# BillyXYB/TransEditor

Measured on AMD Instinct MI355X. Metric: 256x256 images/sec/GPU, G+D fwd+bwd, batch 16; 1/2/4/8-GPU scaling, higher is better.
Workload: dtype f32

## Files before the change

include/te_hip.h:

```cpp
#ifndef TE_HIP_H
#define TE_HIP_H

#include <stdint.h>

#ifdef __cplusplus
extern "C" {
#endif

#define TE_ABI_VERSION 3

#define TE_ERR_NULL -1
#define TE_ERR_SHAPE -2
#define TE_ERR_UNSUPPORTED -3
#define TE_ERR_WORKSPACE -4

typedef void* te_stream_t;

int te_version(void);
const char* te_last_error_string(void);
const char* te_arch(void);

int te_bias_act_f32(float* out, const float* x, const float* b, const float* ref, int act, int grad,
                    float alpha, float scale, int64_t size_x, int64_t step_b, int64_t size_b,
                    te_stream_t stream);
int te_bias_act_f16(void* out, const void* x, const void* b, const void* ref, int act, int grad,
                    float alpha, float scale, int64_t size_x, int64_t step_b, int64_t size_b,
                    te_stream_t stream);
int te_bias_act_f64(double* out, const double* x, const double* b, const double* ref, int act, int grad,
                    float alpha, float scale, int64_t size_x, int64_t step_b, int64_t size_b,
                    te_stream_t stream);

int64_t te_bias_act_bwd_ws_floats(int64_t outer, int64_t C, int64_t inner);
int te_bias_act_bwd_f32(float* gi, float* gb, float* ws, const float* g, const float* ref, float alpha, float scale,
                        int64_t outer, int64_t C, int64_t inner, te_stream_t stream);
int te_bias_act_bwd_rgb_supported(int64_t outer, int64_t C, int64_t inner);
int te_bias_act_bwd_rgb_f32(float* gi, float* gb, float* ws, const float* g, const float* ref, const float* grgb, const float* wrgb,
                            const float* srgb, float wscale, float alpha, float scale, int64_t outer, int64_t C, int64_t inner,
                            te_stream_t stream);

int te_upfirdn2d_f32(float* out, const float* x, const float* k, int64_t major, int in_h, int in_w,
                     int minor, int kh, int kw, int up_x, int up_y, int down_x, int down_y, int pad_x0,
                     int pad_x1, int pad_y0, int pad_y1, const float* b, int64_t size_b, int act,
                     float alpha, float scale, te_stream_t stream);
int te_upfirdn2d_f16(void* out, const void* x, const void* k, int64_t major, int in_h, int in_w,
                     int minor, int kh, int kw, int up_x, int up_y, int down_x, int down_y, int pad_x0,
                     int pad_x1, int pad_y0, int pad_y1, te_stream_t stream);
int te_upfirdn2d_f64(double* out, const double* x, const double* k, int64_t major, int in_h, int in_w,
                     int minor, int kh, int kw, int up_x, int up_y, int down_x, int down_y, int pad_x0,
                     int pad_x1, int pad_y0, int pad_y1, te_stream_t stream);


#define TE_CONV_3X3 0
#define TE_CONV_T2 1
#define TE_CONV_S2 2
#define TE_CONV_1X1 3
#define TE_CONV_3X3W 4
#define TE_CONV_3X3W6 5

#define TE_CONV_S2S6 6

#define TE_CONV_T2S6 7

#define TE_CONV_1X1S6 8

#define TE_PACK_FWD 0
#define TE_PACK_DGRAD 1
#define TE_PACK_SWAP 2
#define TE_PACK_WFWD 3
#define TE_PACK_WDGRAD 4
#define TE_PACK_W6FWD 5
#define TE_PACK_W6DGRAD 6
#define TE_PACK_S6FWD 7
#define TE_PACK_S6SWAP 8
#define TE_PACK_T6FWD 9
#define TE_PACK_T6SWAP 10
#define TE_PACK_P6FWD 11
#define TE_PACK_P6DGRAD 12

int64_t te_conv_packed_numel(int kind_pack, int Co, int Ci, int ksize);
int te_conv_pack_weights_f32(float* wp, const float* w, float wscale, int kind_pack, int Co, int Ci,
                             int ksize, te_stream_t stream);
int te_conv_pack_weights2_f32(float* wp_a, int kind_a, float* wp_b, int kind_b, const float* w, float wscale, int Co, int Ci,
                              int ksize, te_stream_t stream);

int te_conv_pack_weights_multi_f32(int n, float* const* wp, const float* const* w, const float* wscale, const int* kind_pack,
                                   const int* Co, const int* Ci, const int* ksize, te_stream_t stream);

int te_conv_f32(float* out, const float* in, const float* wp, const float* isc, const float* osc,
                const float* bias, int act, int kind, int B, int K, int M, int H, int W,
                te_stream_t stream);
int te_conv_splitk_count(int kind, int B, int K, int M, int H, int W);
int te_conv_wino_supported(int B, int K, int M, int H, int W);
int te_conv_wino6_supported(int B, int K, int M, int H, int W);
int te_conv_s2s6_supported(int B, int K, int M, int H, int W);
int te_conv_t2s6_supported(int B, int K, int M, int H, int W);
int te_conv_p1s6_supported(int B, int K, int M, int H, int W);
int te_conv_wino6_form(int form);
int te_conv_wino6_tiles_per_block(int n);
int te_conv_s2s6_form(int form);
int te_conv_t2s6_form(int form);
int64_t te_conv_t2s6_ws_floats(int B, int K, int H);
int te_conv_ws_f32(float* out, float* ws, const float* in, const float* wp, const float* isc, const float* osc,
                   const float* bias, int act, int kind, int B, int K, int M, int H, int W, te_stream_t stream);
int te_conv_res_f32(float* out, float* ws, const float* in, const float* wp, const float* isc, const float* osc,
                    const float* bias, const float* res, const float* mask_ref, float mask_gain, int act, int kind, int B,
                    int K, int M, int H, int W, te_stream_t stream);

int te_wgrad_slab_count(int kind, int B, int Co, int Ci, int H, int W);
int te_wgrad_pair_form(int kind, int Co, int Ci, int H, int W);
int te_wgrad_split_supported(int kind, int Co, int Ci, int H, int W);
int te_wgrad_split_bf16(int on);
int te_wgrad_t2_wide(int on);
enum { TE_WG6_FP32 = 0, TE_WG6_3X3 = 1, TE_WG6_3X3_PAIR = 2, TE_WG6_T2_WIDE = 3, TE_WG6_T2 = 4, TE_WG6_T2_MASKED = 5, TE_WG6_1X1 = 6 };
int te_wgrad6_form(int kind, int B, int Co, int Ci, int H, int W, int NB);
int te_wgrad_f32(float* slabs, const float* g, const float* x, int kind, int B, int Co, int Ci, int H,
                 int W, int S, te_stream_t stream);
int te_wgrad_group_plan(int kind, int B, int Co, int Ci, int H, int W, int* NB, int* S);
int te_wgrad_group_f32(float* slabs, const float* g, const float* x, int kind, int B, int Co, int Ci, int H, int W, int S, int NB,
                       te_stream_t stream);

int64_t te_wgrad_reduce_ws_floats(int B, int S, int Co, int Ci, int taps, int want_w, int want_isc, int want_osc);
int te_wgrad_reduce_f32(float* gw, float* gisc, float* gosc, float* ws, const float* slabs, const float* w,
                        float wscale, const float* isc, const float* osc, int B, int S, int Co, int Ci,
                        int taps, te_stream_t stream);

int te_rgb_supported(int M, int K, int HW);
int te_rgb_fwd_f32(float* out, const float* x, const float* w, const float* isc, const float* bias, float wscale, int B,
                   int K, int HW, te_stream_t stream);
int te_rgb_dgrad_f32(float* gx, const float* g, const float* w, const float* isc, float wscale, int B, int K, int HW,
                     te_stream_t stream);
int te_rgb_expand_f32(float* out, const float* x3, const float* w, const float* bias, int act, float wscale, int B, int K,
                      int HW, te_stream_t stream);
int te_rgb_wgrad_slab_count(int B, int K, int HW);
int te_rgb_wgrad_f32(float* slabs, const float* g, const float* x, int B, int K, int HW, int S, te_stream_t stream);
int te_rgb_wgrad_sum_f32(float* slabs, const float* g, const float* x, int B, int K, int HW, int S, te_stream_t stream);

int te_attn_fwd_f32(float* o, float* sim, const float* q, const float* k, const float* v, float scale,
                    int N, int G, int M, int L, int D, te_stream_t stream);
int te_attn_bwd_f32(float* gq, float* gk, float* gv, const float* go, const float* gsim_or_null,
                    const float* q, const float* k, const float* v, const float* sim, float scale, int N,
                    int G, int M, int L, int D, te_stream_t stream);

int te_blur_actgrad_tiles(int in_h, int in_w, int kh, int kw, int pad_x0, int pad_x1, int pad_y0, int pad_y1);
int te_blur_actgrad_f32(float* gx, float* partial, const float* g, const float* ref, const float* k, int64_t major, int in_h,
                        int in_w, int kh, int kw, int pad_x0, int pad_x1, int pad_y0, int pad_y1, float alpha, float scale,
                        te_stream_t stream);
int te_blur_gradact_f32(float* gx, float* partial, const float* g, const float* ref, const float* k, int64_t major, int in_h,
                        int in_w, int kh, int kw, int pad_x0, int pad_x1, int pad_y0, int pad_y1, float alpha, float scale,
                        te_stream_t stream);

int te_upfirdn2d_plan(int64_t major, int in_h, int in_w, int minor, int kh, int kw, int up_x, int up_y, int down_x, int down_y,
                      int pad_x0, int pad_x1, int pad_y0, int pad_y1, int* zgroups, int* tiles);
int te_blur_actgrad_plan(int64_t major, int in_h, int in_w, int kh, int kw, int pad_x0, int pad_x1, int pad_y0, int pad_y1,
                         int* zgroups, int* tiles);
int te_blur_gradact_plan(int64_t major, int in_h, int in_w, int kh, int kw, int pad_x0, int pad_x1, int pad_y0, int pad_y1,
                         int* zgroups, int* tiles);
int64_t te_upfirdn2d_direct_cover(int64_t outputs);
int64_t te_chan_scale_cover(int64_t rows, int64_t hw, int aligned16);
int64_t te_bias_act_f32_cover(int64_t size_x, int64_t step_b, int aligned16, int* vec);
int64_t te_bias_act_any_cover(int64_t size_x);
int64_t te_conv_finalize_cover(int64_t outputs);
int64_t te_small_gemm_splitk_finish_cover(int I, int J);
int te_conv_pack_plan(int kind_pack, int Co, int Ci, int ksize, int* blocks, int* tiles);
int te_wgrad_reduce_plan(int B, int S, int Co, int Ci, int taps, int* parts, int64_t* cover);

int te_small_gemm_f32(float* c, float* pre, const float* a, const float* b, const float* bias, const float* residual,
                      float* arowsum, float rs_scale, int I, int J, int K, int64_t sai, int64_t sak, int64_t sbk,
                      int64_t sbj, float alpha, float beta, int act, te_stream_t stream);

int te_small_gemm_splitk_f32(float* c, float* pre, float* ws, int S, const float* a, const float* b, const float* bias,
                             const float* residual, int I, int J, int K, int64_t sai, int64_t sak, int64_t sbk, int64_t sbj,
                             float alpha, float beta, int act, te_stream_t stream);

int te_minibatch_stddev_fwd_f32(float* y, const float* x, int B, int group, int C, int HW, float eps, te_stream_t stream);
int te_minibatch_stddev_bwd_f32(float* gx, const float* gy, const float* x, int B, int group, int C, int HW, float eps,
                                te_stream_t stream);

int te_layer_norm_supported(int64_t R, int N);
int te_layer_norm_fwd_f32(float* y, float* stats, const float* x, int64_t R, int N, float eps, te_stream_t stream);
int te_layer_norm_bwd_f32(float* gx, const float* g, const float* y, const float* stats, int64_t R, int N, te_stream_t stream);

int te_pixel_norm_supported(int64_t B, int D, int C);
int te_pixel_norm_fwd_f32(float* y, float* r, const float* x, int64_t B, int D, int C, float eps, te_stream_t stream);
// ... 114 lines not shown
```

transeditor_amd/_lib.py:

```python
import ctypes as C
import os

import torch

from . import _abi

_HERE = os.path.dirname(os.path.abspath(__file__))
LIB_PATH = os.path.join(_HERE, 'libte_hip.so')
HEADER_PATH = os.path.join(_HERE, '..', 'include', 'te_hip.h')
_lib = _protos = None

CONV_3X3, CONV_T2, CONV_S2, CONV_1X1, CONV_3X3W, CONV_3X3W6, CONV_S2S6, CONV_T2S6, CONV_1X1S6 = 0, 1, 2, 3, 4, 5, 6, 7, 8
(PACK_FWD, PACK_DGRAD, PACK_SWAP, PACK_WFWD, PACK_WDGRAD, PACK_W6FWD, PACK_W6DGRAD, PACK_S6FWD, PACK_S6SWAP, PACK_T6FWD,
 PACK_T6SWAP, PACK_P6FWD, PACK_P6DGRAD) = range(13)


def _header_text():
    if not os.path.exists(HEADER_PATH):
        raise RuntimeError(f'{HEADER_PATH} is missing: the bindings of libte_hip.so are read from it')
    with open(HEADER_PATH) as f:
        return f.read()


def _prototypes():
# ... 195 lines not shown
    B, Cn, H, W = g.shape
    kh, kw = k_flipped.shape
    px0, px1, py0, py1 = pad
    oh, ow = H + py0 + py1 - kh + 1, W + px0 + px1 - kw + 1
    if tuple(ref.shape) != (B, Cn, oh, ow):
        raise RuntimeError(f'blur_gradact: ref {tuple(ref.shape)} is not the shape of the adjoint blur output {(B, Cn, oh, ow)}')
    tiles = lib().te_blur_actgrad_tiles(H, W, kh, kw, px0, px1, py0, py1)
    if tiles <= 0:
        raise RuntimeError(f'te_blur_actgrad_tiles failed ({tiles})')
    gx = torch.empty(B, Cn, oh, ow, device=g.device, dtype=g.dtype)
    partial = torch.empty(B, Cn, tiles, device=g.device, dtype=g.dtype)
    _launch('te_blur_gradact_f32', _ptr(gx), _ptr(partial), _ptr(g), _ptr(ref), _ptr(k_flipped.contiguous()), B * Cn, H, W, kh, kw, px0,
            px1, py0, py1, alpha, scale)
    return gx, partial.sum(dim=(0, 2))


@_op
def conv_pack(w, kind_pack, wscale=1.0):
    w = w.contiguous()
    Co, Ci, ks, _ = w.shape
    n = lib().te_conv_packed_numel(kind_pack, Co, Ci, ks)
    wp = torch.empty(n, device=w.device, dtype=w.dtype)
    _launch('te_conv_pack_weights_f32', _ptr(wp), _ptr(w), wscale, kind_pack, Co, Ci, ks)
    return wp


@_op
def conv_pack2(w, kind_a, kind_b, wscale=1.0):
    w = w.contiguous()
    Co, Ci, ks, _ = w.shape
    wa = torch.empty(lib().te_conv_packed_numel(kind_a, Co, Ci, ks), device=w.device, dtype=w.dtype)
    wb = torch.empty(lib().te_conv_packed_numel(kind_b, Co, Ci, ks), device=w.device, dtype=w.dtype)
    _launch('te_conv_pack_weights2_f32', _ptr(wa), kind_a, _ptr(wb), kind_b, _ptr(w), wscale, Co, Ci, ks)
    return wa, wb


@_op
def conv_pack_multi(jobs):
    n = len(jobs)
    if not n:
        return
    for wp, w, _, _ in jobs:
        if not (w.is_contiguous() and wp.is_contiguous()):
            raise RuntimeError('te_hip: conv_pack_multi needs dense weights and buffers')
    arr = lambda ty, vals: (ty * n)(*vals)
    _launch('te_conv_pack_weights_multi_f32', n, arr(C.c_void_p, [_ptr(j[0]) for j in jobs]), arr(C.c_void_p, [_ptr(j[1]) for j in jobs]),
            arr(C.c_float, [float(j[3]) for j in jobs]), arr(C.c_int, [int(j[2]) for j in jobs]),
            arr(C.c_int, [j[1].shape[0] for j in jobs]), arr(C.c_int, [j[1].shape[1] for j in jobs]),
            arr(C.c_int, [j[1].shape[2] for j in jobs]))


def wino_ok(B, K, M, H, W):
    return bool(lib().te_conv_wino_supported(B, K, M, H, W))


def s2s6_ok(B, K, M, H, W):
    return bool(lib().te_conv_s2s6_supported(B, K, M, H, W))


def t2s6_ok(B, K, M, H, W):
    return bool(lib().te_conv_t2s6_supported(B, K, M, H, W))


def p1s6_ok(B, K, M, H, W):
    return bool(lib().te_conv_p1s6_supported(B, K, M, H, W))


def wino6_form(form=-1):
    return int(lib().te_conv_wino6_form(form))


def wino6_tiles_per_block(n=-1):
    return int(lib().te_conv_wino6_tiles_per_block(n))


def s2s6_form(form=-1):
    return int(lib().te_conv_s2s6_form(form))


def t2s6_form(form=-1):
    return int(lib().te_conv_t2s6_form(form))


def wino6_ok(B, K, M, H, W):
    return bool(lib().te_conv_wino6_supported(B, K, M, H, W))


def conv_out_shape(kind, B, M, H, W):
    if kind in (CONV_T2, CONV_T2S6):
        return (B, M, 2 * H + 1, 2 * W + 1)
    return (B, M, H, W)


@_op
def conv(x, wp, kind, M, H, W, isc=None, osc=None, bias=None, act=0, res=None, mask_ref=None, mask_gain=1.0):
    x = x.contiguous()
    if kind == CONV_1X1S6:
        x = _aligned16(x)
    res = _aligned16(res.contiguous()) if res is not None else None
    mask_ref = _aligned16(mask_ref.contiguous()) if mask_ref is not None else None
    B, K = x.shape[0], x.shape[1]
    out = torch.empty(conv_out_shape(kind, B, M, H, W), device=x.device, dtype=x.dtype)
    if res is not None and tuple(res.shape) != tuple(out.shape):
        raise RuntimeError(f'te_hip: residual {tuple(res.shape)} does not match the convolution output {tuple(out.shape)}')
    if mask_ref is not None and tuple(mask_ref.shape) != tuple(out.shape):
        raise RuntimeError(f'te_hip: mask reference {tuple(mask_ref.shape)} does not match the convolution output {tuple(out.shape)}')
    S = lib().te_conv_splitk_count(kind, B, K, M, H, W)
    if S < 1:
        raise RuntimeError(f'te_conv_splitk_count failed ({S})')
    ws = torch.empty((S,) + tuple(out.shape), device=x.device, dtype=x.dtype) if S > 1 else None
    if kind == CONV_T2S6:
        ws = torch.empty(B * K * H, device=x.device, dtype=x.dtype)
    _launch('te_conv_res_f32', _ptr(out), _ptr(ws), _ptr(x), _ptr(wp), _ptr(isc), _ptr(osc), _ptr(bias), _ptr(res), _ptr(mask_ref),
            mask_gain, act, kind, B, K, M, H, W)
    return out


@_op
def wgrad_slabs(g, x, kind, H, W, group=False):
    g, x = g.contiguous(), x.contiguous()
    B, Co, Ci = g.shape[0], g.shape[1], x.shape[1]
    taps = 1 if kind == CONV_1X1 else 9
    if group:
        nb, sc = C.c_int(0), C.c_int(0)
        _check(lib().te_wgrad_group_plan(kind, B, Co, Ci, H, W, C.byref(nb), C.byref(sc)), 'te_wgrad_group_plan')
        if nb.value > 1:
            slabs = torch.empty(B // nb.value, sc.value, Co, Ci, taps, device=g.device, dtype=g.dtype)
            _launch('te_wgrad_group_f32', _ptr(slabs), _ptr(g), _ptr(x), kind, B, Co, Ci, H, W, sc.value, nb.value)
            return slabs
    S = lib().te_wgrad_slab_count(kind, B, Co, Ci, H, W)
    if S <= 0:
        raise RuntimeError(f'te_wgrad_slab_count failed ({S})')
    slabs = torch.empty(B, S, Co, Ci, taps, device=g.device, dtype=g.dtype)
    _launch('te_wgrad_f32', _ptr(slabs), _ptr(g), _ptr(x), kind, B, Co, Ci, H, W, S)
    return slabs


def wgrad_t2_wide(on=-1):
    return int(lib().te_wgrad_t2_wide(on))


def wgrad_split(on=-1):
    return int(lib().te_wgrad_split_bf16(on))


def wgrad_split_ok(kind, Co, Ci, H, W):
    return bool(lib().te_wgrad_split_supported(kind, Co, Ci, H, W))


WGRAD6_FORMS = ('fp32', 'w6', 'w6pair', 't2wide', 't2narrow', 't2masked', 'p1')


def wgrad6_form(kind, B, Co, Ci, H, W, NB=1):
    return WGRAD6_FORMS[lib().te_wgrad6_form(kind, B, Co, Ci, H, W, NB)]


def wgrad_pair_form(kind, Co, Ci, H, W):
    return bool(lib().te_wgrad_pair_form(kind, Co, Ci, H, W))


@_op
def wgrad_reduce(slabs, w, wscale=1.0, isc=None, osc=None, want_w=True, want_isc=False, want_osc=False):
    B, S, Co, Ci, taps = slabs.shape
    dev, dt = slabs.device, slabs.dtype
    gw = torch.empty(Co, Ci, taps, device=dev, dtype=dt) if want_w else None
    gisc = torch.empty(B, Ci, device=dev, dtype=dt) if want_isc else None
# ... 873 lines not shown
```

transeditor_amd/csrc/s2s6.hip:

```cpp
#include "split6_common.h"
#ifdef S2_PROF
#define TE_PROF
#endif
#include "te_prof.h"

namespace {

constexpr int WT = 512, GT = 256, KC = 16, BM = 64;
constexpr int TH = 8, TWO = 16, PH = 4;
constexpr int IR = 2 * PH + 1, IC = 2 * TWO + 1;
constexpr int CI = 18;
constexpr int NTAP = 9;
constexpr int U_SLOTS = 3 * NTAP * 2;
constexpr int TP_PLANE = IR * 2 * 2 * CI * 4;
constexpr int TP_DWORDS = 3 * TP_PLANE;
constexpr int NG = (IC + 3) / 4;
constexpr int N_ITEMS = IR * NG * 8;
constexpr int P_IN = (N_ITEMS + GT - 1) / GT;
constexpr int N_SLOT = P_IN + 16 * P_IN;
constexpr int SLOT0 = NTAP * 6 - N_SLOT;
constexpr int UA_TAPS = 5;

PROF_BUFFER(s2s6, 2048 * 8 * 8)

struct S2Args {
    float* out; const float* in; const u32x4* U; const float* isc; const float* osc; const float* bias; const float* res;
    const float* mref; float mgain; int act;
    int B, K, M, H, W, Hi, Wi, ntiles, mblocks, tiles_x, tiles_y, nt8;
};


template <bool ISC, bool TWOIMG>
__device__ __attribute__((optnone)) void s2s6_body(const S2Args& p) {
    constexpr int NIMG = TWOIMG ? 2 : 1;
    extern __shared__ __attribute__((aligned(16))) unsigned char smem_raw[];
    u32x4* ul = reinterpret_cast<u32x4*>(smem_raw);
    const int tid = threadIdx.x, lane = tid & 63, l31 = lane & 31, half = lane >> 5;
    const int wid = __builtin_amdgcn_readfirstlane(tid >> 6);
    const int grp = wid >> 2, wq = wid & 3, wm = wq >> 1, wrl = wq & 1, gt = tid & (GT - 1);
    unsigned* tl = reinterpret_cast<unsigned*>(smem_raw + U_SLOTS * 1024) + grp * TP_DWORDS;
    const u32x4* tl4 = reinterpret_cast<const u32x4*>(tl);
    int tile, mbq;
    if (!split6_tile(p.ntiles, p.nt8, p.mblocks, tile, mbq)) return;
    const int tx = tile % p.tiles_x, ty = (tile / p.tiles_x) % p.tiles_y, b = tile / (p.tiles_x * p.tiles_y);
    const int x0 = tx * TWO, y0 = ty * TH, yh = y0 + PH * grp;
    const size_t iplane = (size_t)p.Hi * p.Wi, oplane = (size_t)p.H * p.W;
    const float* inb = p.in + (size_t)b * p.K * iplane;
    const float* iscb = ISC ? p.isc + (size_t)b * p.K : nullptr;

    f32x16 acc[NIMG], accl[NIMG];
#pragma unroll
    for (int m = 0; m < NIMG; ++m)
#pragma unroll
        for (int r = 0; r < 16; ++r) { acc[m][r] = 0.f; accl[m][r] = 0.f; }

    unsigned g_off[P_IN];
    int l_off[P_IN];
    bool last_col[P_IN], live[P_IN];
    unsigned q2[P_IN];
#pragma unroll
    for (int i = 0; i < P_IN; ++i) {
        const int e = gt + GT * i;
        live[i] = e < N_ITEMS;
        const int ee = live[i] ? e : 0;
        const int cg = ee % NG, q = (ee / NG) & 7, row = ee / (NG * 8);
        last_col[i] = cg == NG - 1;
        g_off[i] = (unsigned)((2 * q * p.Hi + 2 * yh + row) * p.Wi + 2 * x0 + 4 * cg - (last_col[i] ? 3 : 0));
        l_off[i] = (((row * 2 + (q >> 2)) * 2) * CI + 2 * cg) * 4 + (q & 3);
        q2[i] = 2u * q;
    }
    const int MT = p.M >> 5;
    f32x4 rin[P_IN][2];
    f32x2 rsc[P_IN];
#pragma unroll
    for (int i = 0; i < P_IN; ++i) rsc[i] = f32x2{1.f, 1.f};
    const int nstage = p.K / KC, nimg = NIMG * nstage;
    auto fetch_scales = [&](int s) {
        if (ISC) {
#pragma unroll
            for (int i = 0; i < P_IN; ++i) rsc[i] = *reinterpret_cast<const f32x2u*>(iscb + s * KC + q2[i]);
        }
    };
    auto fetch_item = [&](int i, int s) {
#pragma unroll
        for (int h2 = 0; h2 < 2; ++h2)
            rin[i][h2] = *reinterpret_cast<const f32x4u*>(inb + ((size_t)s * KC + h2) * iplane + g_off[i]);
    };
    auto issue = [&](int s) {
        fetch_scales(s);
#pragma unroll
        for (int i = 0; i < P_IN; ++i) fetch_item(i, s);
    };
    auto issue_u = [&](int uh, int j) {
        const u32x4* us = p.U + (size_t)(TWOIMG ? j >> 1 : j) * 27 * MT * 64;
        const int mb = TWOIMG ? 2 * mbq + (j & 1) : mbq;
        const int ntap = uh ? NTAP - UA_TAPS : UA_TAPS, tap0 = uh ? UA_TAPS : 0, n = ntap * 6;
#pragma unroll
        for (int r = 0; r < 8; ++r) {
            const int jw = wq + 4 * r;
            if (jw >= n) break;
            const int piece = jw / (ntap * 2), rem = jw % (ntap * 2), tap = tap0 + (rem >> 1), mt = rem & 1;
            const int pt = piece * NTAP + tap;
            const u32x4* g = us + ((size_t)pt * MT + 2 * mb + mt) * 64 + (unsigned)lane;
            __builtin_amdgcn_global_load_lds((const __attribute__((address_space(1))) void*)g,
                                             (__attribute__((address_space(3))) void*)(ul + (pt * 2 + mt) * 64), 16, 0, 0);
        }
    };
    unsigned res[P_IN][4][3];
    float te = 0.f, to = 0.f, fe = 0.f, fo = 0.f;
    auto arith = [&](int k) {
        if (k < 0) {
        } else if (k < P_IN) {
#pragma unroll
            for (int h2 = 0; h2 < 2; ++h2) {
                f32x4 v = rin[k][h2];
                if (last_col[k]) v[0] = v[3];
                rin[k][h2] = ISC ? v * rsc[k][h2] : v;
                asm volatile("" : "+v"(rin[k][h2]));
            }
        } else if (k < N_SLOT) {
            const int u = (k - P_IN) >> 2, j = (k - P_IN) & 3, i = u >> 2, c = u & 3;
            float ve = 0.f, vo = 0.f;
            if (j == 0) {
                ve = rin[i][0][c]; vo = rin[i][1][c];
            }
            split6_step4(j, ve, vo, te, to, fe, fo, res[i][c][0], res[i][c][1], res[i][c][2]);
        }
    };
    auto write_res = [&]() {
#pragma unroll
        for (int i = 0; i < P_IN; ++i) {
            if (!live[i]) continue;
#pragma unroll
            for (int c = 0; c < 4; ++c) {
                if (c > 0 && last_col[i]) continue;
#pragma unroll
                for (int pc = 0; pc < 3; ++pc) tl[l_off[i] + (c & 1) * CI * 4 + (c >> 1) * 4 + pc * TP_PLANE] = res[i][c][pc];
            }
        }
    };
    const int rr = l31 >> 4, jj = l31 & 15;
    const int b_chunk = ((2 * (2 * wrl + rr) * 2 + half) * 2) * CI + jj;
    const int a_chunk = wm * 64 + lane;
    bf16x8 av[2][3], bv[2][3];
    auto rd1 = [&](int t, int slot, int q) {
        const int ky = t / 3, kx = t % 3;
        if (q < 3) av[slot][q] = __builtin_bit_cast(bf16x8, ul[a_chunk + (q * NTAP + t) * 128]);
        else bv[slot][q - 3] = __builtin_bit_cast(bf16x8, tl4[b_chunk + ((ky * 2) * 2 + (kx & 1)) * CI + (kx >> 1) + (q - 3) * (TP_PLANE / 4)]);
    };

    issue(0);
    if (grp == 0) { issue_u(0, 0); issue_u(1, 0); }
#pragma unroll
    for (int k = 0; k < N_SLOT; ++k) arith(k);
    write_res();
    if constexpr (!TWOIMG) {
        issue(1);
        if (grp == 0) {
            if (ISC) asm volatile("s_waitcnt vmcnt(9)" ::: "memory");
            else asm volatile("s_waitcnt vmcnt(6)" ::: "memory");
        }
        split6_barrier();
        const int nphase = 2 * nstage;
        PROF_ONLY(unsigned long long pc[8] = {0, 0, 0, 0, 0, 0, 0, 0};)
        PROF_ONLY(const unsigned long long pstart = __builtin_readcyclecounter(), rstart = __builtin_amdgcn_s_memrealtime();)
        for (int ph = 0; ph < nphase; ++ph) {
            const bool last = ph == nphase - 1;
            PROF_T(t0);
            if ((ph & 1) == grp) {
                const int fs2 = min((ph >> 1) + 2, nstage - 1);
#pragma unroll
                for (int q = 0; q < 6; ++q) rd1(0, 0, q);
                __builtin_amdgcn_s_setprio(1);
#pragma unroll
                for (int t = 0; t < NTAP; ++t) {
                    const int slot = t & 1;
                    if (t == UA_TAPS - 1) { PROF_T(ta); split6_barrier(); PROF_T(tb); PROF_ACC(pc[0], t0, ta); PROF_ACC(pc[1], ta, tb); PROF_ONLY(pc[2] -= tb;) }
                    __builtin_amdgcn_sched_barrier(0);
#pragma unroll
                    for (int q = 0; q < 6; ++q) {
                        split6_product(q, av[slot], bv[slot], acc[0], accl[0]);
                        if (t + 1 < NTAP && q < 3) { rd1(t + 1, slot ^ 1, 2 * q); rd1(t + 1, slot ^ 1, 2 * q + 1); }
                        arith(t * 6 + q - SLOT0);
                        {
                            const int k = t * 6 + q - SLOT0;
                            if (k == P_IN - 1) fetch_scales(fs2);
#pragma unroll
                            for (int i = 0; i < P_IN; ++i)
                                if (k == P_IN + 16 * i + 12) fetch_item(i, fs2);
                        }
                        __builtin_amdgcn_sched_barrier(0);
                    }
                }
                __builtin_amdgcn_s_setprio(0);
                PROF_ONLY({ asm volatile("s_nop 0" ::: "memory"); PROF_T(tc); pc[2] += tc; })
            } else {
                const int cs = (ph + 1) >> 1;
                const bool work = cs >= 1 && cs < nimg;
                if (work && grp == 1) issue_u(1, cs);
                __builtin_amdgcn_sched_barrier(0);
                write_res();
                if (work && grp == 1) split6_wait_vm();
                PROF_T(ta);
                split6_barrier();
                PROF_T(tb);
                if (work && grp == 0) {
                    issue_u(0, cs);
                    split6_wait_vm();
                }
                PROF_T(tc);
                PROF_ACC(pc[3], t0, ta); PROF_ACC(pc[4], ta, tb); PROF_ACC(pc[5], tb, tc);
            }
            PROF_T(t8);
            if (!last) split6_barrier();
            PROF_T(t9);
            PROF_ACC(pc[6], t8, t9);
        }
        PROF_ONLY(if (lane == 0 && blockIdx.x < 2048) {
            unsigned long long* d = te_s2s6_prof_buf + ((size_t)blockIdx.x * 8 + wid) * 8;
            _Pragma("unroll")
            for (int i = 0; i < 6; ++i) d[i] = pc[i];
            d[6] = pc[6] | ((__builtin_amdgcn_s_memrealtime() - rstart) << 40);
            d[7] = ((unsigned long long)nstage << 48) | ((__builtin_readcyclecounter() - pstart) & 0xFFFFFFFFFFFFull);
        })
    } else {
        auto multiply = [&](auto mset_tag, int fs) {
            constexpr int MSET = decltype(mset_tag)::value;
#pragma unroll
            for (int q = 0; q < 6; ++q) rd1(0, 0, q);
            __builtin_amdgcn_s_setprio(1);
#pragma unroll
            for (int t = 0; t < NTAP; ++t) {
                const int slot = t & 1;
                if (t == UA_TAPS - 1) split6_barrier();
                __builtin_amdgcn_sched_barrier(0);
#pragma unroll
                for (int q = 0; q < 6; ++q) {
                    split6_product(q, av[slot], bv[slot], acc[MSET], accl[MSET]);
                    if (t + 1 < NTAP && q < 3) { rd1(t + 1, slot ^ 1, 2 * q); rd1(t + 1, slot ^ 1, 2 * q + 1); }
                    const int k = t * 6 + q;
                    if (MSET == 0) {
                        if (k == 5) fetch_scales(fs);
#pragma unroll
                        for (int i = 0; i < P_IN; ++i)
                            if (k == 6 + 12 * i) fetch_item(i, fs);
                    } else {
                        arith(k - SLOT0);
                    }
                    __builtin_amdgcn_sched_barrier(0);
                }
            }
            __builtin_amdgcn_s_setprio(0);
            split6_barrier();
        };
        auto stage = [&](int ph, bool write) {
            const int cs = (ph + 1) >> 1;
            const bool work = cs >= 1 && cs < nimg;
            if (grp == 1 && work) issue_u(1, cs);
            __builtin_amdgcn_sched_barrier(0);
            if (write) write_res();
            if (grp == 1 && work) split6_wait_vm();
            split6_barrier();
            if (grp == 0 && work) {
                issue_u(0, cs);
                split6_wait_vm();
            }
            split6_barrier();
        };
        split6_wait_vm();
        split6_barrier();
        int ph = 0;
        if (grp == 1) { stage(0, false); ph = 1; }
        for (int s = 0; s < nstage; ++s) {
            const int fs = min(s + 1, nstage - 1);
            multiply(std::integral_constant<int, 0>{}, fs);
            stage(ph + 1, false);
            multiply(std::integral_constant<int, 1>{}, fs);
            if (!(grp == 1 && s == nstage - 1)) stage(ph + 3, true);
            ph += 4;
        }
    }

    const float g_pos = p.act == 3 ? 1.4142135623730951f : 1.f;
#pragma unroll
    for (int m = 0; m < NIMG; ++m) {
        const int mbase = (NIMG * mbq + m) * BM + wm * 32;
        const size_t off0 = ((size_t)b * p.M + mbase) * oplane + (size_t)(yh + 2 * wrl + rr) * p.W + x0 + jj;
        float scv[16], biv[16], resv[16], mrefv[16];
#pragma unroll
        for (int r = 0; r < 16; ++r) {
            const int dm = (r & 3) + 8 * (r >> 2) + 4 * half;
            scv[r] = p.osc ? p.osc[(size_t)b * p.M + mbase + dm] : 1.f;
            biv[r] = p.bias ? p.bias[mbase + dm] : 0.f;
        }
        if (p.res) {
#pragma unroll
            for (int r = 0; r < 16; ++r) resv[r] = p.res[off0 + (size_t)((r & 3) + 8 * (r >> 2) + 4 * half) * oplane];
        }
        if (p.mref) {
#pragma unroll
            for (int r = 0; r < 16; ++r) mrefv[r] = p.mref[off0 + (size_t)((r & 3) + 8 * (r >> 2) + 4 * half) * oplane];
        }
#pragma unroll
        for (int r = 0; r < 16; ++r) {
            const int dm = (r & 3) + 8 * (r >> 2) + 4 * half;
            float v = (acc[m][r] + accl[m][r]) * scv[r] + biv[r];
            if (p.act >= 3) v = (v > 0.f ? v : v * 0.2f) * g_pos;
            if (p.res) v += resv[r];
            if (p.mref) v *= mrefv[r] > 0.f ? p.mgain : 0.2f * p.mgain;
            p.out[off0 + (size_t)dm * oplane] = v;
        }
    }
}

template <bool ISC>
__global__ __launch_bounds__(WT, 2) void s2s6_kernel(const S2Args p) { [[clang::always_inline]] s2s6_body<ISC, false>(p); }
template <bool ISC>
__global__ __launch_bounds__(WT, 2) void s2s6q_kernel(const S2Args p) { [[clang::always_inline]] s2s6_body<ISC, true>(p); }

}

PROF_READBACK(s2s6)

extern "C" int te_conv_s2s6_supported(int B, int K, int M, int H, int W) {
    if (!(B > 0 && K >= 32 && K % KC == 0 && M >= BM && M % BM == 0 && H >= TH && H % TH == 0 && W >= TWO && W % TWO == 0)) return 0;
    return ((int64_t)K * (2 * H + 1) * (2 * W + 1) * 4 < 0x7FFFFFFF && (int64_t)B * (H / TH) * (W / TWO) * (M / BM) < 0x7FFFFFF0) ? 1 : 0;
}

static std::atomic<int> g_s2_form{1};
extern "C" int te_conv_s2s6_form(int form) {
    const int old = g_s2_form.load(std::memory_order_relaxed);
    if (form >= 0 && form <= 2) g_s2_form.store(form, std::memory_order_relaxed);
    return old;
}

int te_s2s6_launch(float* out, const float* in, const float* U, const float* isc, const float* osc, const float* bias, const float* res,
                   const float* mask_ref, float mask_gain, int act, int B, int K, int M, int H, int W, hipStream_t s) {
    TE_REQUIRE(te_conv_s2s6_supported(B, K, M, H, W), TE_ERR_UNSUPPORTED,
               "te_conv_f32(TE_CONV_S2S6): needs K %% 16 == 0 (>= 32), M %% 64 == 0, H %% 8 == 0, W %% 16 == 0 (te_conv_s2s6_supported)");
    TE_REQUIRE((reinterpret_cast<uintptr_t>(U) & 15) == 0 && (reinterpret_cast<uintptr_t>(in) & 3) == 0, TE_ERR_UNSUPPORTED,
               "te_conv_f32(TE_CONV_S2S6): 16-byte aligned packed weights required");
    S2Args a{};
    a.out = out; a.in = in; a.U = reinterpret_cast<const u32x4*>(U); a.isc = isc; a.osc = osc; a.bias = bias; a.res = res;
    a.mref = mask_ref; a.mgain = mask_gain; a.act = act;
    a.B = B; a.K = K; a.M = M; a.H = H; a.W = W; a.Hi = 2 * H + 1; a.Wi = 2 * W + 1;
    a.tiles_x = W / TWO; a.tiles_y = H / TH; a.mblocks = M / BM;
    a.ntiles = B * a.tiles_x * a.tiles_y;
    a.nt8 = te::xcd_banded() ? (int)te::cdiv(a.ntiles, 8) : 0;
    const int64_t blocks = te::cdiv(a.ntiles, 8) * 8 * a.mblocks;
    const size_t lds = (size_t)U_SLOTS * 1024 + 2 * (size_t)TP_DWORDS * 4;
    const int form = g_s2_form.load(std::memory_order_relaxed);
    const int64_t blocks_q = te::cdiv(a.ntiles, 8) * 8 * (M / (2 * BM));
    if (split6_two_image(form, M, blocks_q)) {
        a.mblocks = M / (2 * BM);
        SPLIT6_LAUNCH_ISC(s2s6q_kernel, isc, dim3((unsigned)blocks_q), WT, lds, s, a);
    } else {
        SPLIT6_LAUNCH_ISC(s2s6_kernel, isc, dim3((unsigned)blocks), WT, lds, s, a);
    }
    return te::launch_status("te_conv_f32(TE_CONV_S2S6)");
}
```

transeditor_amd/csrc/split6_common.h:

```cpp
#pragma once
#include "conv_common.h"

typedef short bf16x8 __attribute__((ext_vector_type(8)));
typedef __bf16 bf16x2 __attribute__((ext_vector_type(2)));
typedef float f32x2 __attribute__((ext_vector_type(2)));
typedef float f32x2u __attribute__((ext_vector_type(2), aligned(4)));
typedef float f32x4u __attribute__((ext_vector_type(4), aligned(4)));
typedef unsigned u32x4 __attribute__((ext_vector_type(4)));

__device__ __forceinline__ void split6_barrier() { asm volatile("s_waitcnt lgkmcnt(0)\n\ts_barrier" ::: "memory"); }
__device__ __forceinline__ void split6_wait_vm() { asm volatile("s_waitcnt vmcnt(0)" ::: "memory"); }

__device__ __forceinline__ unsigned split6_piece(float te, float to) {
    const f32x2 t = {te, to};
    return __builtin_bit_cast(unsigned, __builtin_convertvector(t, bf16x2));
}
__device__ __forceinline__ unsigned split6_take(float te, float to, float& fe, float& fo) {
    const unsigned h = split6_piece(te, to);
    fe = __builtin_bit_cast(float, h << 16);
    fo = __builtin_bit_cast(float, h & 0xFFFF0000u);
    return h;
}
__device__ __forceinline__ void split6_pin(float& te, float& to, float& fe, float& fo) { asm volatile("" : "+v"(te), "+v"(to), "+v"(fe), "+v"(fo)); }
template <bool PIN_LOW = true>
__device__ __forceinline__ void split6_step4(int j, float ve, float vo, float& te, float& to, float& fe, float& fo, unsigned& h, unsigned& m, unsigned& l) {
    if (j == 0) {
        te = ve; to = vo;
        h = split6_take(te, to, fe, fo);
    } else if (j == 1) {
        te -= fe; to -= fo;
    } else if (j == 2) {
        m = split6_take(te, to, fe, fo);
    } else {
        te -= fe; to -= fo;
        l = split6_piece(te, to);
        if (PIN_LOW) asm volatile("" : "+v"(l));
    }
    split6_pin(te, to, fe, fo);
}
__device__ __forceinline__ void split6_step3(int j, float ve, float vo, float& te, float& to, float& fe, float& fo, unsigned& h, unsigned& m, unsigned& l) {
    if (j == 0) {
        te = ve; to = vo;
        h = split6_take(te, to, fe, fo);
    } else if (j == 1) {
        te -= fe; to -= fo;
        m = split6_take(te, to, fe, fo);
    } else {
        te -= fe; to -= fo;
        l = split6_piece(te, to);
    }
    split6_pin(te, to, fe, fo);
}

__device__ __forceinline__ void split6_product(int q, const bf16x8 (&a)[3], const bf16x8 (&b)[3], f32x16& big, f32x16& small) {
    constexpr int PA[6] = {1, 0, 2, 0, 1, 0}, PB[6] = {1, 2, 0, 1, 0, 0};
    f32x16& d = q < 5 ? small : big;
    d = __builtin_amdgcn_mfma_f32_32x32x16_bf16(a[PA[q]], b[PB[q]], d, 0, 0, 0);
}

__device__ __forceinline__ bool split6_tile(int ntiles, int nt8, int mblocks, int& tile, int& mb) {
    const int xcd = blockIdx.x & 7, jx = blockIdx.x >> 3;
    const int tq = jx / mblocks;
    mb = jx % mblocks;
    tile = nt8 ? (int)(((int64_t)xcd * ntiles) >> 3) + tq : tq * 8 + xcd;
    return tile < (nt8 ? (int)(((int64_t)(xcd + 1) * ntiles) >> 3) : ntiles);
}

__device__ __forceinline__ bool split6_tile_list(int ntiles, int nt8, int mblocks, int lists, int& tile, int& end, int& step, int& mb) {
    step = nt8 ? 1 : 8;
    if (lists == 0) {
        const bool has = split6_tile(ntiles, nt8, mblocks, tile, mb);
        end = tile + step;
        return has;
    }
    const int xcd = blockIdx.x & 7, jx = blockIdx.x >> 3;
    const int lq = jx / mblocks;
    mb = jx % mblocks;
    const int first = nt8 ? (int)(((int64_t)xcd * ntiles) >> 3) : xcd;
    const int nb = nt8 ? (int)(((int64_t)(xcd + 1) * ntiles) >> 3) - first : (ntiles - xcd + 7) >> 3;
    const int lo = (int)((int64_t)lq * nb / lists), hi = (int)((int64_t)(lq + 1) * nb / lists);
    tile = first + step * lo;
    end = first + step * hi;
    return lo < hi;
}


inline bool split6_two_image(int form_sel, int M, int64_t blocks_q) { return form_sel >= 1 && M % 128 == 0 && (form_sel == 2 || blocks_q >= te::kNumCU); }

template <auto KERNEL, class Args>
inline void split6_launch(dim3 grid, int threads, size_t lds, hipStream_t s, const Args& a) {
    static std::atomic<uint64_t> attr_done{0};
    te::allow_big_lds(attr_done, (const void*)KERNEL, 160 * 1024);
    KERNEL<<<grid, threads, lds, s>>>(a);
}
#define SPLIT6_LAUNCH_ISC(kernel, isc, blocks, threads, lds, s, a) \
    ((isc) ? split6_launch<kernel<true>>(blocks, threads, lds, s, a) : split6_launch<kernel<false>>(blocks, threads, lds, s, a))
```

transeditor_amd/csrc/wino6.hip:

```cpp
#include "split6_common.h"
#include "wino6_schedule.h"
#ifdef W6P_PROF
#define TE_PROF
#endif
#include "te_prof.h"

namespace {

constexpr int WT = 512, KC = 16, TW = 32, NP = TW / 2, BM = 64, TH = 8;
constexpr int U_CHUNKS = 36 * 2 * 64;

struct Wino6Args {
    float* out; const float* in; const u32x4* U; const float* isc; const float* osc; const float* bias; const float* res;
    const float* mref; float mgain; int act;
    int B, K, M, H, W, ntiles, mblocks, tiles_x, tiles_y, nt8;
    int lists;
    int lgpw;
};

constexpr int PH = 4, PR = PH + 2;
constexpr int TP_PLANE = PR * 2 * NP * 4;
constexpr int TP_DWORDS = 12 * TP_PLANE;
constexpr int GT = WT / 2;
constexpr int P_IN = (PR * NP * 8) / GT;
// ... 469 lines not shown
        asm volatile("" : "+v"(elane));
        const int ehalf = elane >> 5, err = (elane & 31) >> 4, ejj = elane & 15;
        const int wr = grp * 2 + wrl;
        const int eM = e->M, eW = e->W, eact = e->act;
        const size_t eplane = (size_t)e->H * eW;
        const float emgain = e->mgain;
        const float g_pos = eact == 3 ? 1.4142135623730951f : 1.f;
        float* const eout = e->out;
        const float* const eosc = e->osc; const float* const ebias = e->bias; const float* const eres = e->res; const float* const emref = e->mref;
#pragma unroll
        for (int m = 0; m < 2; ++m) {
            const int mbase = (2 * mbq + m) * BM + wm * 32;
            const size_t off0 = ((size_t)b * eM + mbase) * eplane + (size_t)(y0 + 2 * wr) * eW + x0;
            const unsigned lo = (unsigned)(err * eW + 2 * ejj) + 4u * (unsigned)ehalf * (unsigned)eplane;
#pragma unroll
            for (int r0 = 0; r0 < 16; r0 += 4) {
                float scv[4], biv[4];
#pragma unroll
                for (int r = r0; r < r0 + 4; ++r) {
                    const int mm = mbase + (r & 3) + 8 * (r >> 2) + 4 * ehalf;
                    scv[r - r0] = eosc ? eosc[(size_t)b * eM + mm] : 1.f;
                    biv[r - r0] = ebias ? ebias[mm] : 0.f;
                }
                f32x2 resv[4], mrefv[4];
                if (eres) {
#pragma unroll
                    for (int r = r0; r < r0 + 4; ++r)
                        resv[r - r0] = *reinterpret_cast<const f32x2*>(eres + off0 + (size_t)((r & 3) + 8 * (r >> 2)) * eplane + lo);
                }
                if (emref) {
#pragma unroll
                    for (int r = r0; r < r0 + 4; ++r)
                        mrefv[r - r0] = *reinterpret_cast<const f32x2*>(emref + off0 + (size_t)((r & 3) + 8 * (r >> 2)) * eplane + lo);
                }
#pragma unroll
                for (int r = r0; r < r0 + 4; ++r) {
                    float v0 = acc[m][0][r] + acc[m][1][r] + acc[m][2][r];
                    float v1 = acc[m][1][r] - acc[m][2][r] - acc[m][3][r];
                    const float sc = scv[r - r0], bi = biv[r - r0];
                    v0 = v0 * sc + bi;
                    v1 = v1 * sc + bi;
                    if (eact >= 3) {
                        v0 = (v0 > 0.f ? v0 : v0 * 0.2f) * g_pos;
                        v1 = (v1 > 0.f ? v1 : v1 * 0.2f) * g_pos;
                    }
                    if (eres) { v0 += resv[r - r0][0]; v1 += resv[r - r0][1]; }
                    if (emref) {
                        v0 *= mrefv[r - r0][0] > 0.f ? emgain : 0.2f * emgain;
                        v1 *= mrefv[r - r0][1] > 0.f ? emgain : 0.2f * emgain;
                    }
                    f32x2 v; v[0] = v0; v[1] = v1;
                    *reinterpret_cast<f32x2*>(eout + off0 + (size_t)((r & 3) + 8 * (r >> 2)) * eplane + lo) = v;
                }
            }
        }
        if (!has_next) break;
        tile += tile_step;
#pragma unroll
        for (int m = 0; m < 2; ++m)
#pragma unroll
            for (int c = 0; c < 4; ++c)
#pragma unroll
                for (int r = 0; r < 16; ++r) acc[m][c][r] = 0.f;
    }
}

}

static std::atomic<int> g_w6_form{2};
extern "C" int te_conv_wino6_form(int form) {
    const int old = g_w6_form.load(std::memory_order_relaxed);
    if (form >= 1 && form <= 3) g_w6_form.store(form, std::memory_order_relaxed);
    return old;
}

constexpr int W6_MAX_TPB = 4096;
static std::atomic<int> g_w6_tpb{0};
extern "C" int te_conv_wino6_tiles_per_block(int n) {
    const int old = g_w6_tpb.load(std::memory_order_relaxed);
    if (n >= 0 && n <= W6_MAX_TPB) g_w6_tpb.store(n, std::memory_order_relaxed);
    return old;
}

static int w6_auto_tpb(int nt8c, int mblocks) {
    const int64_t rounds1 = te::cdiv((int64_t)8 * nt8c * mblocks, te::kNumCU);
    for (int n = 4; n >= 2; --n) {
        const int64_t blocks = (int64_t)8 * te::cdiv(nt8c, n) * mblocks;
        if (blocks >= te::kNumCU && te::cdiv(blocks, te::kNumCU) * n <= rounds1) return n;
    }
    return 1;
}

PROF_READBACK(w6p)

extern "C" int te_conv_wino6_supported(int B, int K, int M, int H, int W) {
    if (!(B > 0 && K >= 32 && K % 32 == 0 && M >= BM && M % BM == 0 && H >= TH && H % TH == 0)) return 0;
    const bool wide = W >= TW && W % TW == 0, pair16 = W == 16 && B % 2 == 0;
    if (!wide && !pair16) return 0;
    const int64_t tiles = wide ? (int64_t)B * (H / TH) * (W / TW) : (int64_t)(B / 2) * (H / TH);
    if (!wide && tiles * (M / BM) < te::kNumCU / 2) return 0;
    return ((int64_t)K * H * W * 4 * (wide ? 1 : 2) < 0x7FFFFFFF && tiles * (M / BM) < 0x7FFFFFF0) ? 1 : 0;
}

int te_wino6_launch(float* out, const float* in, const float* U, const float* isc, const float* osc, const float* bias, const float* res,
                    const float* mask_ref, float mask_gain, int act, int B, int K, int M, int H, int W, hipStream_t s) {
    TE_REQUIRE(te_conv_wino6_supported(B, K, M, H, W), TE_ERR_UNSUPPORTED,
               "te_conv_f32(TE_CONV_3X3W6): needs K %% 32 == 0, M %% 64 == 0, W %% 32 == 0 (or W == 16 and an even batch), H %% 8 == 0 (te_conv_wino6_supported)");
    TE_REQUIRE(((reinterpret_cast<uintptr_t>(out) | reinterpret_cast<uintptr_t>(U) | reinterpret_cast<uintptr_t>(res) |
                 reinterpret_cast<uintptr_t>(mask_ref)) & 15) == 0 && (reinterpret_cast<uintptr_t>(in) & 3) == 0, TE_ERR_UNSUPPORTED,
               "te_conv_f32(TE_CONV_3X3W6): 16-byte aligned tensors required");
    Wino6Args a{};
    a.out = out; a.in = in; a.U = reinterpret_cast<const u32x4*>(U); a.isc = isc; a.osc = osc; a.bias = bias; a.res = res;
    a.mref = mask_ref; a.mgain = mask_gain; a.act = act;
    a.B = B; a.K = K; a.M = M; a.H = H; a.W = W;
    a.lgpw = W >= TW ? 4 : 3;
    a.tiles_x = W >= TW ? W / TW : 1; a.tiles_y = H / TH; a.mblocks = M / BM;
    a.ntiles = (W >= TW ? B : B / 2) * a.tiles_x * a.tiles_y;
    a.nt8 = te::xcd_banded() ? (int)te::cdiv(a.ntiles, 8) : 0;
    const int64_t blocks = te::cdiv(a.ntiles, 8) * 8 * a.mblocks;
    const int form = g_w6_form.load(std::memory_order_relaxed);
    const int64_t blocks_q = te::cdiv(a.ntiles, 8) * 8 * (M / (2 * BM));
    if (W >= TW && split6_two_image(form - 1, M, blocks_q)) {
        a.mblocks = M / (2 * BM);
        const int nt8c = (int)te::cdiv(a.ntiles, 8);
        int tpb = g_w6_tpb.load(std::memory_order_relaxed);
        if (tpb == 0) tpb = w6_auto_tpb(nt8c, a.mblocks);
        a.lists = tpb >= 2 ? (int)te::cdiv(nt8c, tpb) : 0;
        const int64_t blocks2 = a.lists ? (int64_t)8 * a.lists * a.mblocks : blocks_q;
        const size_t lds = (size_t)U_CHUNKS * 16 + 2 * (size_t)TP_DWORDS * 4;
        SPLIT6_LAUNCH_ISC(wino6q_kernel, isc, dim3((unsigned)blocks2), WT, lds, s, a);
    } else {
        const size_t lds = (size_t)U_CHUNKS * 16 + 2 * (size_t)TP_DWORDS * 4;
        SPLIT6_LAUNCH_ISC(wino6p_kernel, isc, dim3((unsigned)blocks), WT, lds, s, a);
    }
    return te::launch_status("te_conv_f32(TE_CONV_3X3W6)");
}
```

Measured before the change: 150.7.

## Make stride-2 split6 conv kernel walk multiple tiles per block with cross-tile prefetch

The two-image s2s6 kernel becomes persistent over a list of tiles, reusing the wino6 schedule helpers. It prefetches the next tile's input while the current tile's multiplies finish, then runs a per-tile epilogue. This removes per-block launch, prologue and pipeline-fill cost and evens out the tail across CUs. The price is more kernel complexity and register pressure, the per-tile epilogue reading kernel args again, and a shared auto tiles-per-block heuristic now used by both kernels.

```diff
diff --git a/include/te_hip.h b/include/te_hip.h
--- a/include/te_hip.h
+++ b/include/te_hip.h
@@ -99,6 +99,7 @@
 int te_conv_wino6_tiles_per_block(int n);
 int te_conv_s2s6_form(int form);
 int te_conv_t2s6_form(int form);
+int te_conv_s2s6_tiles_per_block(int n);
 int64_t te_conv_t2s6_ws_floats(int B, int K, int H);
 int te_conv_ws_f32(float* out, float* ws, const float* in, const float* wp, const float* isc, const float* osc,
                    const float* bias, int act, int kind, int B, int K, int M, int H, int W, te_stream_t stream);
diff --git a/transeditor_amd/_lib.py b/transeditor_amd/_lib.py
--- a/transeditor_amd/_lib.py
+++ b/transeditor_amd/_lib.py
@@ -301,6 +301,10 @@
     return int(lib().te_conv_t2s6_form(form))
 
 
+def s2s6_tiles_per_block(n=-1):
+    return int(lib().te_conv_s2s6_tiles_per_block(n))
+
+
 def wino6_ok(B, K, M, H, W):
     return bool(lib().te_conv_wino6_supported(B, K, M, H, W))
 
diff --git a/transeditor_amd/csrc/s2s6.hip b/transeditor_amd/csrc/s2s6.hip
--- a/transeditor_amd/csrc/s2s6.hip
+++ b/transeditor_amd/csrc/s2s6.hip
@@ -1,4 +1,5 @@
 #include "split6_common.h"
+#include "wino6_schedule.h"
 #ifdef S2_PROF
 #define TE_PROF
 #endif
@@ -27,6 +28,7 @@
     float* out; const float* in; const u32x4* U; const float* isc; const float* osc; const float* bias; const float* res;
     const float* mref; float mgain; int act;
     int B, K, M, H, W, Hi, Wi, ntiles, mblocks, tiles_x, tiles_y, nt8;
+    int lists;
 };
 
 
@@ -40,13 +42,11 @@
     const int grp = wid >> 2, wq = wid & 3, wm = wq >> 1, wrl = wq & 1, gt = tid & (GT - 1);
     unsigned* tl = reinterpret_cast<unsigned*>(smem_raw + U_SLOTS * 1024) + grp * TP_DWORDS;
     const u32x4* tl4 = reinterpret_cast<const u32x4*>(tl);
-    int tile, mbq;
-    if (!split6_tile(p.ntiles, p.nt8, p.mblocks, tile, mbq)) return;
-    const int tx = tile % p.tiles_x, ty = (tile / p.tiles_x) % p.tiles_y, b = tile / (p.tiles_x * p.tiles_y);
-    const int x0 = tx * TWO, y0 = ty * TH, yh = y0 + PH * grp;
-    const size_t iplane = (size_t)p.Hi * p.Wi, oplane = (size_t)p.H * p.W;
-    const float* inb = p.in + (size_t)b * p.K * iplane;
-    const float* iscb = ISC ? p.isc + (size_t)b * p.K : nullptr;
+    int tile, tile_end, tile_step, mbq;
+    if (!split6_tile_list(p.ntiles, p.nt8, p.mblocks, TWOIMG ? p.lists : 0, tile, tile_end, tile_step, mbq)) return;
+    const size_t iplane = (size_t)p.Hi * p.Wi;
+    const float* inb;
+    const float* iscb = nullptr;
 
     f32x16 acc[NIMG], accl[NIMG];
 #pragma unroll
@@ -58,6 +58,29 @@
     int l_off[P_IN];
     bool last_col[P_IN], live[P_IN];
     unsigned q2[P_IN];
+    typedef const __attribute__((address_space(4))) S2Args* KArgs;
+    auto kargs = [&]() {
+        KArgs k = (KArgs)__builtin_amdgcn_kernarg_segment_ptr();
+        if (TWOIMG) asm volatile("" : "+s"(k));
+        return k;
+    };
+    auto set_tile = [&](int t) {
+        const KArgs a = kargs();
+        const int aHi = a->Hi, aWi = a->Wi, atx = a->tiles_x, aty = a->tiles_y, aK = a->K;
+        const int tx = t % atx, ty = (t / atx) % aty, b = t / (atx * aty);
+        const int x0 = tx * TWO, yh = ty * TH + PH * grp;
+        inb = a->in + (size_t)b * aK * ((size_t)aHi * aWi);
+        if (ISC) iscb = a->isc + (size_t)b * aK;
+        int gto = gt;
+        if (TWOIMG) asm volatile("" : "+v"(gto));
+#pragma unroll
+        for (int i = 0; i < P_IN; ++i) {
+            const int e = gto + GT * i, ee = e < N_ITEMS ? e : 0;
+            const int cg = ee % NG, q = (ee / NG) & 7, row = ee / (NG * 8);
+            g_off[i] = (unsigned)((2 * q * aHi + 2 * yh + row) * aWi + 2 * x0 + 4 * cg - (cg == NG - 1 ? 3 : 0));
+        }
+    };
+    set_tile(tile);
 #pragma unroll
     for (int i = 0; i < P_IN; ++i) {
         const int e = gt + GT * i;
@@ -65,7 +88,6 @@
         const int ee = live[i] ? e : 0;
         const int cg = ee % NG, q = (ee / NG) & 7, row = ee / (NG * 8);
         last_col[i] = cg == NG - 1;
-        g_off[i] = (unsigned)((2 * q * p.Hi + 2 * yh + row) * p.Wi + 2 * x0 + 4 * cg - (last_col[i] ? 3 : 0));
         l_off[i] = (((row * 2 + (q >> 2)) * 2) * CI + 2 * cg) * 4 + (q & 3);
         q2[i] = 2u * q;
     }
@@ -95,9 +117,11 @@
         const u32x4* us = p.U + (size_t)(TWOIMG ? j >> 1 : j) * 27 * MT * 64;
         const int mb = TWOIMG ? 2 * mbq + (j & 1) : mbq;
         const int ntap = uh ? NTAP - UA_TAPS : UA_TAPS, tap0 = uh ? UA_TAPS : 0, n = ntap * 6;
+        int wqo = wq;
+        if (TWOIMG) asm volatile("" : "+s"(wqo));
 #pragma unroll
         for (int r = 0; r < 8; ++r) {
-            const int jw = wq + 4 * r;
+            const int jw = wqo + 4 * r;
             if (jw >= n) break;
             const int piece = jw / (ntap * 2), rem = jw % (ntap * 2), tap = tap0 + (rem >> 1), mt = rem & 1;
             const int pt = piece * NTAP + tap;
@@ -147,6 +171,53 @@
         const int ky = t / 3, kx = t % 3;
         if (q < 3) av[slot][q] = __builtin_bit_cast(bf16x8, ul[a_chunk + (q * NTAP + t) * 128]);
         else bv[slot][q - 3] = __builtin_bit_cast(bf16x8, tl4[b_chunk + ((ky * 2) * 2 + (kx & 1)) * CI + (kx >> 1) + (q - 3) * (TP_PLANE / 4)]);
+    };
+
+    auto epilogue = [&](int t) {
+        const KArgs e = kargs();
+        const int tx = t % e->tiles_x, ty = (t / e->tiles_x) % e->tiles_y, b = t / (e->tiles_x * e->tiles_y);
+        const int x0 = tx * TWO, yh = ty * TH + PH * grp;
+        int elane = lane;
+        asm volatile("" : "+v"(elane));
+        const int ehalf = elane >> 5, err = (elane & 31) >> 4, ejj = elane & 15;
+        const int eM = e->M, eW = e->W, eact = e->act;
+        const size_t eplane = (size_t)e->H * eW;
+        const float emgain = e->mgain;
+        const float g_pos = eact == 3 ? 1.4142135623730951f : 1.f;
+        float* const eout = e->out;
+        const float* const eosc = e->osc; const float* const ebias = e->bias; const float* const eres = e->res; const float* const emref = e->mref;
+#pragma unroll
+        for (int m = 0; m < NIMG; ++m) {
+            const int mbase = (NIMG * mbq + m) * BM + wm * 32;
+            const size_t off0 = ((size_t)b * eM + mbase) * eplane + (size_t)(yh + 2 * wrl) * eW + x0;
+            const unsigned lo = (unsigned)(err * eW + ejj) + 4u * (unsigned)ehalf * (unsigned)eplane;
+#pragma unroll
+            for (int r0 = 0; r0 < 16; r0 += 4) {
+                float scv[4], biv[4], resv[4], mrefv[4];
+#pragma unroll
+                for (int r = r0; r < r0 + 4; ++r) {
+                    const int mm = mbase + (r & 3) + 8 * (r >> 2) + 4 * ehalf;
+                    scv[r - r0] = eosc ? eosc[(size_t)b * eM + mm] : 1.f;
+                    biv[r - r0] = ebias ? ebias[mm] : 0.f;
+                }
+                if (eres) {
+#pragma unroll
+                    for (int r = r0; r < r0 + 4; ++r) resv[r - r0] = eres[off0 + (size_t)((r & 3) + 8 * (r >> 2)) * eplane + lo];
+                }
+                if (emref) {
+#pragma unroll
+                    for (int r = r0; r < r0 + 4; ++r) mrefv[r - r0] = emref[off0 + (size_t)((r & 3) + 8 * (r >> 2)) * eplane + lo];
+                }
+#pragma unroll
+                for (int r = r0; r < r0 + 4; ++r) {
+                    float v = (acc[m][r] + accl[m][r]) * scv[r - r0] + biv[r - r0];
+                    if (eact >= 3) v = (v > 0.f ? v : v * 0.2f) * g_pos;
+                    if (eres) v += resv[r - r0];
+                    if (emref) v *= mrefv[r - r0] > 0.f ? emgain : 0.2f * emgain;
+                    eout[off0 + (size_t)((r & 3) + 8 * (r >> 2)) * eplane + lo] = v;
+                }
+            }
+        }
     };
 
     issue(0);
@@ -253,38 +324,53 @@
             __builtin_amdgcn_s_setprio(0);
             split6_barrier();
         };
-        auto stage = [&](int ph, bool write) {
-            const int cs = (ph + 1) >> 1;
-            const bool work = cs >= 1 && cs < nimg;
-            if (grp == 1 && work) issue_u(1, cs);
+        auto stage = [&](int ph, bool write, bool has_next) {
+            const int cs = wino6_sched::renew_image(ph);
+            const bool work = wino6_sched::renew_work(cs, nimg, has_next);
+            const int ci = cs == nimg ? 0 : cs;
+            if (grp == 1 && work) issue_u(1, ci);
             __builtin_amdgcn_sched_barrier(0);
             if (write) write_res();
             if (grp == 1 && work) split6_wait_vm();
             split6_barrier();
             if (grp == 0 && work) {
-                issue_u(0, cs);
+                issue_u(0, ci);
                 split6_wait_vm();
             }
             split6_barrier();
         };
         split6_wait_vm();
         split6_barrier();
-        int ph = 0;
-        if (grp == 1) { stage(0, false); ph = 1; }
-        for (int s = 0; s < nstage; ++s) {
-            const int fs = min(s + 1, nstage - 1);
-            multiply(std::integral_constant<int, 0>{}, fs);
-            stage(ph + 1, false);
-            multiply(std::integral_constant<int, 1>{}, fs);
-            if (!(grp == 1 && s == nstage - 1)) stage(ph + 3, true);
-            ph += 4;
+        for (;;) {
+            const bool has_next = tile + tile_step < tile_end;
+            int ph = 0;
+            if (wino6_sched::lead_phase(grp)) { stage(0, false, has_next); ph = 1; }
+            for (int s = 0; s < nstage; ++s) {
+                bool next_tile;
+                const int fs = wino6_sched::fetch_stage(s, nstage, has_next, next_tile);
+                if (next_tile) set_tile(tile + tile_step);
+                multiply(std::integral_constant<int, 0>{}, fs);
+                stage(ph + 1, false, has_next);
+                multiply(std::integral_constant<int, 1>{}, fs);
+                if (wino6_sched::runs_sb(grp, s, nstage, has_next)) stage(ph + 3, true, has_next);
+                ph += 4;
+            }
+            for (int i = 0; i < wino6_sched::tail_barriers(grp, has_next); ++i) split6_barrier();
+            epilogue(tile);
+            if (!has_next) break;
+            tile += tile_step;
+#pragma unroll
+            for (int m = 0; m < NIMG; ++m)
+#pragma unroll
+                for (int r = 0; r < 16; ++r) { acc[m][r] = 0.f; accl[m][r] = 0.f; }
         }
     }
-
-    const float g_pos = p.act == 3 ? 1.4142135623730951f : 1.f;
-#pragma unroll
-    for (int m = 0; m < NIMG; ++m) {
-        const int mbase = (NIMG * mbq + m) * BM + wm * 32;
+    if constexpr (!TWOIMG) {
+        const int tx = tile % p.tiles_x, ty = (tile / p.tiles_x) % p.tiles_y, b = tile / (p.tiles_x * p.tiles_y);
+        const int x0 = tx * TWO, yh = ty * TH + PH * grp;
+        const size_t oplane = (size_t)p.H * p.W;
+        const float g_pos = p.act == 3 ? 1.4142135623730951f : 1.f;
+        const int mbase = mbq * BM + wm * 32;
         const size_t off0 = ((size_t)b * p.M + mbase) * oplane + (size_t)(yh + 2 * wrl + rr) * p.W + x0 + jj;
         float scv[16], biv[16], resv[16], mrefv[16];
 #pragma unroll
@@ -304,7 +390,7 @@
 #pragma unroll
         for (int r = 0; r < 16; ++r) {
             const int dm = (r & 3) + 8 * (r >> 2) + 4 * half;
-            float v = (acc[m][r] + accl[m][r]) * scv[r] + biv[r];
+            float v = (acc[0][r] + accl[0][r]) * scv[r] + biv[r];
             if (p.act >= 3) v = (v > 0.f ? v : v * 0.2f) * g_pos;
             if (p.res) v += resv[r];
             if (p.mref) v *= mrefv[r] > 0.f ? p.mgain : 0.2f * p.mgain;
@@ -333,6 +419,17 @@
     if (form >= 0 && form <= 2) g_s2_form.store(form, std::memory_order_relaxed);
     return old;
 }
+
+constexpr int S2_MAX_TPB = 4096;
+static std::atomic<int> g_s2_tpb{0};
+extern "C" int te_conv_s2s6_tiles_per_block(int n) {
+    const int old = g_s2_tpb.load(std::memory_order_relaxed);
+    if (n >= 0 && n <= S2_MAX_TPB) g_s2_tpb.store(n, std::memory_order_relaxed);
+    return old;
+}
+
+constexpr int S2_AUTO_TPB = 4;
+static int s2_auto_tpb(int nt8c, int mblocks) { return split6_auto_tpb(nt8c, mblocks, S2_AUTO_TPB); }
 
 int te_s2s6_launch(float* out, const float* in, const float* U, const float* isc, const float* osc, const float* bias, const float* res,
                    const float* mask_ref, float mask_gain, int act, int B, int K, int M, int H, int W, hipStream_t s) {
@@ -353,7 +450,11 @@
     const int64_t blocks_q = te::cdiv(a.ntiles, 8) * 8 * (M / (2 * BM));
     if (split6_two_image(form, M, blocks_q)) {
         a.mblocks = M / (2 * BM);
-        SPLIT6_LAUNCH_ISC(s2s6q_kernel, isc, dim3((unsigned)blocks_q), WT, lds, s, a);
+        const int nt8c = (int)te::cdiv(a.ntiles, 8);
+        int tpb = g_s2_tpb.load(std::memory_order_relaxed);
+        if (tpb == 0) tpb = s2_auto_tpb(nt8c, a.mblocks);
+        const int64_t blocks2 = split6_walk_grid(tpb, nt8c, a.mblocks, blocks_q, a.lists);
+        SPLIT6_LAUNCH_ISC(s2s6q_kernel, isc, dim3((unsigned)blocks2), WT, lds, s, a);
     } else {
         SPLIT6_LAUNCH_ISC(s2s6_kernel, isc, dim3((unsigned)blocks), WT, lds, s, a);
     }
diff --git a/transeditor_amd/csrc/split6_common.h b/transeditor_amd/csrc/split6_common.h
--- a/transeditor_amd/csrc/split6_common.h
+++ b/transeditor_amd/csrc/split6_common.h
@@ -87,6 +87,19 @@
 
 inline bool split6_two_image(int form_sel, int M, int64_t blocks_q) { return form_sel >= 1 && M % 128 == 0 && (form_sel == 2 || blocks_q >= te::kNumCU); }
 
+inline int split6_auto_tpb(int nt8c, int mblocks, int nmax) {
+    const int64_t rounds1 = te::cdiv((int64_t)8 * nt8c * mblocks, te::kNumCU);
+    for (int n = nmax; n >= 2; --n) {
+        const int64_t blocks = (int64_t)8 * te::cdiv(nt8c, n) * mblocks;
+        if (blocks >= te::kNumCU && te::cdiv(blocks, te::kNumCU) * n <= rounds1) return n;
+    }
+    return 1;
+}
+inline int64_t split6_walk_grid(int tpb, int nt8c, int mblocks, int64_t blocks_q, int& lists) {
+    lists = tpb >= 2 ? (int)te::cdiv(nt8c, tpb) : 0;
+    return lists ? (int64_t)8 * lists * mblocks : blocks_q;
+}
+
 template <auto KERNEL, class Args>
 inline void split6_launch(dim3 grid, int threads, size_t lds, hipStream_t s, const Args& a) {
     static std::atomic<uint64_t> attr_done{0};
diff --git a/transeditor_amd/csrc/wino6.hip b/transeditor_amd/csrc/wino6.hip
--- a/transeditor_amd/csrc/wino6.hip
+++ b/transeditor_amd/csrc/wino6.hip
@@ -575,14 +575,7 @@
     return old;
 }
 
-static int w6_auto_tpb(int nt8c, int mblocks) {
-    const int64_t rounds1 = te::cdiv((int64_t)8 * nt8c * mblocks, te::kNumCU);
-    for (int n = 4; n >= 2; --n) {
-        const int64_t blocks = (int64_t)8 * te::cdiv(nt8c, n) * mblocks;
-        if (blocks >= te::kNumCU && te::cdiv(blocks, te::kNumCU) * n <= rounds1) return n;
-    }
-    return 1;
-}
+static int w6_auto_tpb(int nt8c, int mblocks) { return split6_auto_tpb(nt8c, mblocks, 4); }
 
 PROF_READBACK(w6p)
 
```

Result: no change. 151.0 (median of 6 runs) (+0.2%).
